# quanpn90/avsr

Measured on AMD Instinct MI355X. Metric: AV-frames/sec/GPU (fwd+bwd) on 15s clips; WER parity on LRS2 test, higher is better.
Workload: dtype bf16

## Files before the change

### avsr_amd/csrc/conv.hip

```cpp
#include "gemm_core.h"
#include "gemm_glds.h"

using namespace gemmcore;

namespace {

static int ilog2(int v) { int s = 0; while ((1 << s) < v) ++s; return (1 << s) == v ? s : -1; }

static int make_geom(const avsr_conv_params* p, ConvGeom& g) {
  g.nimg = p->nimg; g.hin = p->hin; g.win = p->win; g.hout = p->hout; g.wout = p->wout;
  g.kh = p->kh; g.kw = p->kw; g.sh = p->sh; g.sw = p->sw; g.ph = p->ph; g.pw = p->pw;
  g.cin = p->cin; g.cout = p->cout; g.ldx = p->ldx; g.ldy = p->ldy;
  g.f_hw_out = make_fastdiv((uint32_t)(p->hout * p->wout));
  g.f_w_out = make_fastdiv((uint32_t)p->wout);
  g.f_hw_in = make_fastdiv((uint32_t)(p->hin * p->win));
  g.f_w_in = make_fastdiv((uint32_t)p->win);
  g.f_kw = make_fastdiv((uint32_t)p->kw);
  g.cin_shift = ilog2(p->cin); g.cout_shift = ilog2(p->cout);
  g.ktot_w = p->kh * p->kw * p->cin; g.tap_kfw = p->kw; g.tap_kh0 = 0; g.tap_kw0 = 0; g.tap_step = 1;
  const int ve = p->dtype == AVSR_BF16 ? 8 : 4;
  if (g.cin_shift < 0 || g.cout_shift < 0 || p->cin < ve || p->cout < ve) return AVSR_E_SHAPE;
  if (p->ldx % ve || p->ldy % ve) return AVSR_E_ALIGN;
  if (p->groups < 1 || p->ldx < (int64_t)p->groups * p->cin || p->ldy < (int64_t)p->groups * p->cout) return AVSR_E_SHAPE;
  return 0;
}

struct ConvArgs {
  ConvGeom g;
  uint32_t a_bytes, b_bytes;
  const void* a; const void* b;
  int64_t a_gstride, b_gstride, c_gstride;
  int M, N, K, splits, kchunk;
  float* ws;
  Epi e;
  gemmg::BnrArgs bnr;
};

enum { K_FWD = 0, K_DGRAD = 1, K_WGRAD = 2, K_DGRAD_BNR = 3 };

template <typename T, typename OutT, int WM, int WN, int KIND>
__global__ __launch_bounds__(NT) void conv_kernel(ConvArgs a) {
  extern __shared__ __attribute__((aligned(16))) char smem[];
  using TL = Tile<T, WM, WN>;
  const int z = blockIdx.z, grp = z / a.splits, sp = z % a.splits;
  const int m0 = blockIdx.y * TL::BM, n0 = blockIdx.x * TL::BN;
  const T* pa = (const T*)a.a + (int64_t)grp * a.a_gstride;
  const T* pb = (const T*)a.b + (int64_t)grp * a.b_gstride;
  f32x16 acc[2][2];
  const int kbeg = sp * a.kchunk, kend = min(a.K, kbeg + a.kchunk);
  if constexpr (KIND == K_FWD) {
    LdConvK<T, TL::BM, false> la; la.p = pa; la.g = a.g; la.rext = a.M; la.K = a.K;
    LdDenseK<T, TL::BN> lb; lb.p = pb; lb.ld = a.K; lb.rext = a.N; lb.K = a.K;
    mainloop<T, WM, WN>(la, lb, m0, n0, kbeg, kend, acc, smem);
  } else if constexpr (KIND == K_DGRAD) {
    LdConvK<T, TL::BM, true> la; la.p = pa; la.g = a.g; la.rext = a.M; la.K = a.K;
    LdWgtR<T, TL::BN> lb; lb.p = pb; lb.g = a.g; lb.rext = a.N; lb.K = a.K;
    mainloop<T, WM, WN>(la, lb, m0, n0, kbeg, kend, acc, smem);
  } else {
    LdDenseR<T, TL::BM> la; la.p = pa; la.ld = a.g.ldy; la.rext = a.M; la.K = a.K;
    LdConvR<T, TL::BN> lb; lb.p = pb; lb.g = a.g; lb.rext = a.N; lb.K = a.K;
    mainloop<T, WM, WN>(la, lb, m0, n0, kbeg, kend, acc, smem);
  }
  Epi e = a.e;
  if (KIND == K_WGRAD && a.ws) e.C = a.ws + ((int64_t)grp * a.splits + sp) * a.M * a.N;
  else e.C = (OutT*)e.C + (int64_t)grp * a.c_gstride;
  if (e.res) e.res = (const T*)e.res + (int64_t)grp * a.c_gstride;
  if (e.preact) e.preact = (T*)e.preact + (int64_t)grp * a.c_gstride;
  if (e.bias) e.bias += (int64_t)grp * a.c_gstride;
  epilogue<T, OutT, WM, WN>(e, m0, n0, acc, smem);
}

using gemmg::GBK;
using gemmg::glds16;
using gemmg::g_zero_line;

template <int R, int NW, bool TRANSP> struct GConvK {
  static constexpr bool KMAJ = true;
  static constexpr int SLOTS = R / 8 / NW;
  const bf16* p; ConvGeom g; int kend;
  int pn[SLOTS], ph_[SLOTS], pw_[SLOTS], kc[SLOTS];
  AVSR_DEV void init(const bf16* base, const ConvGeom& g_, int r0, int rext, int kend_, int wave, int lane) {
    p = base; g = g_; kend = kend_;
#pragma unroll
    for (int i = 0; i < SLOTS; ++i) {
      const int pc = i * NW + wave, pr = pc * 8 + (lane >> 3);
      kc[i] = ((lane & 7) ^ ((pr >> 1) & 7)) * 8;
      const int r = r0 + pr;
      if (r >= rext) { pn[i] = 0; ph_[i] = -1000000; pw_[i] = 0; continue; }
      if (!TRANSP) {
        uint32_t n = fdiv(r, g.f_hw_out); uint32_t rem = r - n * g.f_hw_out.d;
        uint32_t oh = fdiv(rem, g.f_w_out); uint32_t ow = rem - oh * g.f_w_out.d;
        pn[i] = n * g.hin * g.win; ph_[i] = oh * g.sh - g.ph; pw_[i] = ow * g.sw - g.pw;
      } else {
        uint32_t n = fdiv(r, g.f_hw_in); uint32_t rem = r - n * g.f_hw_in.d;
        uint32_t h = fdiv(rem, g.f_w_in); uint32_t w = rem - h * g.f_w_in.d;
        pn[i] = n * g.hout * g.wout; ph_[i] = h + g.ph; pw_[i] = w + g.pw;
      }
    }
  }
  AVSR_DEV void issue(char* img, int k0, int wave) const {
    const int cs = TRANSP ? g.cout_shift : g.cin_shift;
#pragma unroll
    for (int i = 0; i < SLOTS; ++i) {
      const int k = k0 + kc[i];
      const int c = k & ((1 << cs) - 1), khw = k >> cs;
      const int kh = fdiv(khw, g.f_kw), kw = khw - kh * g.f_kw.d;
      bool ok = k < kend;
      int64_t off;
      if (!TRANSP) {
        const int ih = ph_[i] + kh, iw = pw_[i] + kw;
        ok = ok && ih >= 0 && ih < g.hin && iw >= 0 && iw < g.win;
        off = (int64_t)(pn[i] + ih * g.win + iw) * g.ldx + c;
      } else {
        const int th = ph_[i] - kh, tw = pw_[i] - kw;
        const int oh = th / g.sh, ow = tw / g.sw;
        ok = ok && th >= 0 && tw >= 0 && oh * g.sh == th && ow * g.sw == tw && oh < g.hout && ow < g.wout;
        off = (int64_t)(pn[i] + oh * g.wout + ow) * g.ldy + c;
      }
      glds16(ok ? (const void*)(p + off) : (const void*)g_zero_line, img + (i * NW + wave) * 1024);
    }
  }
};

template <int R, int NW> struct GWgtR {
  static constexpr bool KMAJ = false;
  static constexpr int CPR = R / 8, RPP = 64 / CPR, SLOTS = GBK / RPP / NW;
  const bf16* p; ConvGeom g; int kend;
  int kr[SLOTS], rr[SLOTS];
  AVSR_DEV void init(const bf16* base, const ConvGeom& g_, int r0, int rext, int kend_, int wave, int lane) {
    p = base; g = g_; kend = kend_;
#pragma unroll
    for (int i = 0; i < SLOTS; ++i) {
      const int pc = i * NW + wave, pk = pc * RPP + lane / CPR;
      const int c = (lane % CPR) ^ gemmg::rswz<CPR>(pk);
      kr[i] = pk;
      rr[i] = r0 + c * 8 < rext ? r0 + c * 8 : -1;
    }
  }
  AVSR_DEV void issue(char* img, int k0, int wave) const {
    const int ktot = g.kh * g.kw * g.cin;
#pragma unroll
    for (int i = 0; i < SLOTS; ++i) {
      const int k = k0 + kr[i];
      const int co = k & ((1 << g.cout_shift) - 1), khw = k >> g.cout_shift;
      const bool ok = k < kend && rr[i] >= 0;
      glds16(ok ? (const void*)(p + (int64_t)co * ktot + khw * g.cin + rr[i]) : (const void*)g_zero_line,
             img + (i * NW + wave) * 1024);
    }
  }
};

template <int R, int NW> struct GConvR {
  static constexpr bool KMAJ = false;
  static constexpr int CPR = R / 8, RPP = 64 / CPR, SLOTS = GBK / RPP / NW;
// ... 357 lines not shown
    k.nkw = k.kw0 < p->kw ? (p->kw - k.kw0 + 1) / 2 : 0;
    k.ci = (k.a + p->ph - k.kh0) / 2; k.cj = (k.b + p->pw - k.kw0) / 2;
  }
}

static bool s2_phase(const avsr_conv_params* p) {
  if (!avsr_opt(AVSR_OPT_CONV_S2PHASE)) return false;
  if (p->sh != 2 || p->sw != 2 || p->groups != 1 || p->dtype != AVSR_BF16 || !conv_glds_enabled()) return false;
  if (p->cout % 64) return false;
  ConvArgs t;
  set_extents(t, p, true, ((int64_t)p->nimg * p->hout * p->wout - 1) * p->ldy + p->cout,
              (int64_t)p->cout * p->kh * p->kw * p->cin);
  return t.a_bytes != 0;
}

struct PatchGeom {
  int nimg, H, W, Wp, PP;
  FastDiv f_pp, f_wp, f_hw, f_w;
  int sign;
};
constexpr int PATCH_ROWS = 384;
constexpr int PATCH_BYTES = PATCH_ROWS * 128;
using PCfg = gemmg::GCfg<4, 1, 2, 2, 3>;
constexpr int PATCH_SB = PCfg::BN * GBK * 2;
constexpr int PATCH_LDS = PATCH_BYTES + PCfg::S * PATCH_SB;
static_assert(PCfg::EP_BYTES <= PATCH_LDS && PCfg::NTH * 33 * 4 <= PATCH_LDS, "epilogue staging exceeds LDS");

AVSR_DEV int patch_pos(int p, const PatchGeom& pg) {
  const uint32_t n = fdiv((uint32_t)p, pg.f_hw), rem = (uint32_t)p - n * pg.f_hw.d;
  const uint32_t y = fdiv(rem, pg.f_w), x = rem - y * pg.f_w.d;
  return (int)(n * pg.PP + (y + 1) * pg.Wp + x + 1);
}

template <int NW> struct PatchLoad {
  static constexpr int PIECES = PATCH_ROWS * 8 / 64 / NW;
  __amdgpu_buffer_rsrc_t rs;
  uint32_t vo[PIECES];
  AVSR_DEV void init(const bf16* base, uint32_t bytes, const PatchGeom& pg, int qmin, int wave, int lane) {
    rs = make_rsrc(base, bytes);
#pragma unroll
    for (int i = 0; i < PIECES; ++i) {
      const int pr = (i * NW + wave) * 8 + (lane >> 3);
      const int c = (lane & 7) ^ ((pr >> 1) & 7);
      const uint32_t q = (uint32_t)(qmin + pr);
      const uint32_t n = fdiv(q, pg.f_pp), rem = q - n * (uint32_t)pg.PP;
      const uint32_t yy = fdiv(rem, pg.f_wp), xx = rem - yy * (uint32_t)pg.Wp;
      const bool ok = n < (uint32_t)pg.nimg && yy - 1u < (uint32_t)pg.H && xx - 1u < (uint32_t)pg.W;
      vo[i] = ok ? (((n * pg.H + yy - 1) * pg.W + xx - 1) * 64u + c * 8u) * 2u : OOB;
    }
  }
  AVSR_DEV void issue(char* img, int wave) const {
#pragma unroll
    for (int i = 0; i < PIECES; ++i) bglds16(rs, vo[i], 0u, img + (i * NW + wave) * 1024);
  }
};

template <class LB>
struct PatchFrags {
  bf16x8 a[PCfg::TM], b[PCfg::TN];
  AVSR_DEV void load(const char* patch, const int (&row)[PCfg::TM], int toff, const char* wstage, int s, int lane) {
#pragma unroll
    for (int i = 0; i < PCfg::TM; ++i) {
      const int r = row[i] + toff;
      const int c = (4 * s + (lane >> 4)) ^ ((r >> 1) & 7);
      a[i] = *(const bf16x8*)(patch + r * 128 + c * 16);
    }
#pragma unroll
    for (int j = 0; j < PCfg::TN; ++j) b[j] = gemmg::gfrag<PCfg::BN, LB::KMAJ>(wstage, j * 16, s, lane);
  }
  AVSR_DEV void mma(f32x4 (&acc)[PCfg::TM][PCfg::TN]) const {
#pragma unroll
    for (int i = 0; i < PCfg::TM; ++i)
#pragma unroll
      for (int j = 0; j < PCfg::TN; ++j) acc[i][j] = mfma16(a[i], b[j], acc[i][j]);
  }
};

template <int KIND>
__global__ __launch_bounds__(PCfg::NTH, 2) void conv_patch_kernel(ConvArgs a, PatchGeom pg) {
  extern __shared__ __attribute__((aligned(16))) char smem[];
  constexpr int S = PCfg::S, NK = 9, KS = GBK / 32, GLB = PATCH_SB / 1024 / PCfg::NW;
  const int m0 = gemmg::xcd_remap(blockIdx.x, gridDim.x) * PCfg::BM;
  const int lane = threadIdx.x & 63, wave = __builtin_amdgcn_readfirstlane(threadIdx.x >> 6);
  const int qmin = patch_pos(m0, pg) - pg.Wp - 1;
  char* patch = smem;
  char* ring = smem + PATCH_BYTES;
  PatchLoad<PCfg::NW> lp;
  lp.init((const bf16*)a.a, a.a_bytes, pg, qmin, wave, lane);
  using LB = typename std::conditional<KIND == K_FWD, gemmg::BDenseK<PCfg::BN, PCfg::NW>,
                                       BWgtR<PCfg::BN, PCfg::NW>>::type;
  LB lb;
  if constexpr (KIND == K_FWD) lb.init((const bf16*)a.b, a.b_bytes, a.K, 0, a.N, a.K, wave, lane);
  else lb.init((const bf16*)a.b, a.b_bytes, a.g, 0, a.N, wave, lane);
  int row[PCfg::TM];
#pragma unroll
  for (int i = 0; i < PCfg::TM; ++i) {
    const int p = min(m0 + wave * 64 + i * 16 + (lane & 15), a.M - 1);
    row[i] = patch_pos(p, pg) - qmin;
  }
  f32x4 acc[PCfg::TM][PCfg::TN];
#pragma unroll
  for (int i = 0; i < PCfg::TM; ++i)
#pragma unroll
    for (int j = 0; j < PCfg::TN; ++j) acc[i][j] = f32x4{0.f, 0.f, 0.f, 0.f};
  lp.issue(patch, wave);
#pragma unroll
  for (int p = 0; p < S; ++p) lb.issue(ring + p * PATCH_SB, p * GBK, wave);
  gemmg::wait_vmcnt<GLB * (S - 1)>();
  __builtin_amdgcn_s_barrier();
  asm volatile("" ::: "memory");
  auto toff = [&](int kt) {
    const int kh = kt / 3, kw = kt - 3 * kh;
    return pg.sign * ((kh - 1) * pg.Wp + (kw - 1));
  };
  static_assert(KS == 2, "the fragment sets alternate over two k-steps per K-tile");
  PatchFrags<LB> f0, f1;
  f0.load(patch, row, toff(0), ring, 0, lane);
  int cs = 0;
  for (int kt = 0; kt < NK; ++kt) {
    const int ns = cs + 1 == S ? 0 : cs + 1;
    f1.load(patch, row, toff(kt), ring + cs * PATCH_SB, 1, lane);
    f0.mma(acc);
    if (kt + 1 < NK) {
      asm volatile("s_waitcnt lgkmcnt(0)" ::: "memory");
      if (kt + S - 1 < NK) gemmg::wait_vmcnt<GLB * (S - 2)>();
      else gemmg::wait_vmcnt<0>();
      __builtin_amdgcn_s_barrier();
      asm volatile("" ::: "memory");
      if (kt + S < NK) lb.issue(ring + cs * PATCH_SB, (kt + S) * GBK, wave);
      f0.load(patch, row, toff(kt + 1), ring + ns * PATCH_SB, 0, lane);
    }
    f1.mma(acc);
    cs = ns;
  }
  __syncthreads();
  if constexpr (KIND >= K_DGRAD_BNR) {
    gemmg::epilogue_bnr<PCfg, KIND - K_DGRAD_BNR>(a.e, a.bnr, m0, 0, acc, smem);
  } else {
    gemmg::epilogue_g<bf16, bf16, PCfg>(a.e, m0, 0, acc, smem);
  }
}

#ifndef AVSR_WP_BLOCKS
#define AVSR_WP_BLOCKS 128
#endif
#ifndef AVSR_WP34
#define AVSR_WP34 1
#endif
#ifndef AVSR_WP34_BLOCKS
#define AVSR_WP34_BLOCKS 128
#endif
constexpr int WP_BLOCKS = AVSR_WP_BLOCKS, WP34_BLOCKS = AVSR_WP34_BLOCKS, WP_COLS = 576;

template <int W_, int TR_, int TPI_, int NBUF_, int PST_, int IPT_ = 1, int NBLK_ = WP_BLOCKS, int SPREAD_ = 0>
struct WPGeo {
  static constexpr int W = W_, TR = TR_, TPI = TPI_, H = TR * TPI, NBUF = NBUF_, PST = PST_, IPT = IPT_, NBLK = NBLK_;
  static constexpr int IMGT = TR * W;
  static constexpr int PX = IPT * IMGT;
  static constexpr int KS = (PX + 31) / 32;
  static constexpr int DYR = KS * 32;
  static constexpr int WP = W + 2, PROWS = (IPT * (TR + 1) + 1) * WP;
  static constexpr int SLOTS = PST / 16;
  static constexpr int PPIECE = (PROWS * SLOTS + 255) / 256;
  static constexpr int PBYTES = PPIECE * 4 * 1024;
  static constexpr int DYPIECE = DYR * 128 / 4096;
  static constexpr int DYB = DYR * 128;
  static constexpr int BUF = DYB + PBYTES;
  static constexpr int LDS = NBUF * BUF;
  static constexpr int NP = DYPIECE + PPIECE;
  static constexpr int SPREAD = SPREAD_ > 0 ? SPREAD_ : KS;
  static_assert(LDS <= 160 * 1024, "the tile buffers must fit the CU's LDS");
  static_assert(IPT == 1 || TPI == 1, "a tile is part of one image or whole images");
  static_assert(NBUF >= 2 && (NBUF - 2) * NP <= 63 && SPREAD <= KS, "vmcnt range / DMA spread");
  static_assert(NBLK % 8 == 0, "blocks come in XCD groups of 8");
};
using WPStage1 = WPGeo<22, 11, 2, 2, 144>;
using WPStage2 = WPGeo<11, 11, 1, 3, 160>;
using WPStage3 = WPGeo<6, 6, 1, 2, 144, 5, WP34_BLOCKS, 3>;
using WPStage4 = WPGeo<3, 3, 1, 2, 160, 14, WP34_BLOCKS, 2>;

AVSR_DEV int whswz(int row) { return ((row >> 1) & 3) << 1; }
AVSR_DEV bf16x8 trpair(const char* pa, const char* pb) {
  const v4i16 a = __builtin_amdgcn_ds_read_tr16_b64_v4i16((lds_v4i16*)pa);
  const v4i16 b = __builtin_amdgcn_ds_read_tr16_b64_v4i16((lds_v4i16*)pb);
  union { v4i16 s4[2]; bf16x8 h; } u;
  u.s4[0] = a; u.s4[1] = b;
  return u.h;
}

AVSR_DEV void wp_block(int b, int nq, int nblk, int& q, int& r) {
  const int x = b & 7, s = b >> 3, S = nblk >> 3;
  if (nq <= S) {
    q = s % nq;
    r = (s / nq) * 8 + x;
  } else {
    const int k = nq / S;
    r = x / k;
    q = (x - r * k) * S + s;
  }
}

template <int NP, int K>
AVSR_DEV void wp_wait_ahead(int ahead) {
  if constexpr (K == 0) {
    gemmg::wait_vmcnt<0>();
  } else {
    if (ahead >= K) gemmg::wait_vmcnt<NP * K>();
    else wp_wait_ahead<NP, K - 1>(ahead);
  }
}

template <class G>
__global__ __launch_bounds__(256, 1) void conv_wgrad_patch_kernel(const bf16* __restrict__ x, const bf16* __restrict__ dy,
                                                                  uint32_t x_bytes, uint32_t dy_bytes, int nimg,
                                                                  int cin, int cout, float* __restrict__ ws) {
  extern __shared__ __attribute__((aligned(16))) char smem[];
  constexpr int IMG = G::H * G::W;
  const int lane = threadIdx.x & 63, wave = __builtin_amdgcn_readfirstlane(threadIdx.x >> 6);
  const int ncih = cin / 64, nq = (cout / 64) * ncih, bpq = gridDim.x / nq;
  int q, rng;
  wp_block(blockIdx.x, nq, gridDim.x, q, rng);
  const int coh = q / ncih, cih = q - coh * ncih;
  const int ntiles = (nimg * G::TPI + G::IPT - 1) / G::IPT;
  const int ta = (int)((int64_t)ntiles * rng / bpq), tb = (int)((int64_t)ntiles * (rng + 1) / bpq);
  const __amdgpu_buffer_rsrc_t rx = make_rsrc(x, x_bytes), rdy = make_rsrc(dy, dy_bytes);
  auto tile_px = [&](int t) { return (t / G::TPI) * IMG * G::IPT + (t % G::TPI) * G::PX; };
  auto issue_dy = [&](int i, int t, char* buf) {
    const int s = (wave + 4 * i) * 64 + lane, row = s >> 3;
    const int c = (s & 7) ^ whswz(row);
    const uint32_t vo = row < G::PX ? (uint32_t)(tile_px(t) + row) * (uint32_t)(cout * 2) + coh * 128 + c * 16 : gemmg::OOB;
    gemmg::bglds16(rdy, vo, 0u, buf + (wave + 4 * i) * 1024);
  };
  auto issue_patch = [&](int i, int t, char* buf) {
    const int s = (wave + 4 * i) * 64 + lane, row = s / G::SLOTS, ch = s - row * G::SLOTS;
    const int py = row / G::WP, pxp = row - py * G::WP;
    bool ok;
    int src;
    if constexpr (G::IPT == 1) {
      const int y = (t % G::TPI) * G::TR + py - 1;
      ok = y >= 0 && y < G::H;
      src = (py - 1) * G::W + pxp - 1;
    } else {
      const int i = (py - 1) / (G::TR + 1), yl = py - 1 - i * (G::TR + 1);
      ok = py >= 1 && yl < G::TR;
      src = i * G::IMGT + yl * G::W + pxp - 1;
    }
    ok = ok && ch < 8 && row < G::PROWS && pxp >= 1 && pxp <= G::W;
    const uint32_t vo = ok ? (uint32_t)(tile_px(t) + src) * (uint32_t)(cin * 2) + cih * 128 + ch * 16 : gemmg::OOB;
    gemmg::bglds16(rx, vo, 0u, buf + G::DYB + (wave + 4 * i) * 1024);
  };
  const int g = lane >> 4, qq = (lane & 15) >> 2, pp = lane & 3;
  const int pxa = 16 * (g >> 1) + 4 * (g & 1) + qq;
  const int sw = whswz(pxa);
  int dA[4];
#pragma unroll
  for (int i = 0; i < 4; ++i) dA[i] = pxa * 128 + (((2 * i + (pp >> 1)) ^ sw) << 4) + 8 * (pp & 1);
  auto prow = [&](int px) {
    px = min(px, G::PX - 1);
    const int i = px / G::IMGT, r = px - i * G::IMGT, yy = r / G::W, xx = r - yy * G::W;
    return (i * (G::TR + 1) + yy + 1) * G::WP + xx + 1;
  };
  int pA[G::KS], pB[G::KS];
#pragma unroll
  for (int kb = 0; kb < G::KS; ++kb) {
    pA[kb] = (prow(32 * kb + pxa) - G::WP - 1) * G::PST + 32 * wave + 8 * pp;
    pB[kb] = (prow(32 * kb + pxa + 8) - G::WP - 1) * G::PST + 32 * wave + 8 * pp;
  }
  f32x4 acc[4][9];
#pragma unroll
  for (int i = 0; i < 4; ++i)
#pragma unroll
    for (int t = 0; t < 9; ++t) acc[i][t] = f32x4{0.f, 0.f, 0.f, 0.f};
  constexpr int PD = G::NBUF - 1;
#pragma unroll
  for (int d = 0; d < PD; ++d)
    if (ta + d < tb) {
#pragma unroll
      for (int i = 0; i < G::DYPIECE; ++i) issue_dy(i, ta + d, smem + d * G::BUF);
#pragma unroll
      for (int i = 0; i < G::PPIECE; ++i) issue_patch(i, ta + d, smem + d * G::BUF);
    }
  constexpr int PER = (G::NP + G::SPREAD - 1) / G::SPREAD;
  for (int t = ta; t < tb; ++t) {
    const char* buf = smem + ((t - ta) % G::NBUF) * G::BUF;
    char* nbuf = smem + ((t + PD - ta) % G::NBUF) * G::BUF;
    const bool more = t + PD < tb;
    wp_wait_ahead<G::NP, PD - 1>(tb - 1 - t);
    __builtin_amdgcn_s_barrier();
    asm volatile("" ::: "memory");
    const char* patch = buf + G::DYB;
    struct Fr { bf16x8 a[4], b[9]; };
    auto load = [&](Fr& f, int kb) {
#pragma unroll
      for (int i = 0; i < 4; ++i) f.a[i] = trpair(buf + dA[i] + kb * 4096, buf + dA[i] + kb * 4096 + 1024);
#pragma unroll
      for (int tp = 0; tp < 9; ++tp) {
        const int off = ((tp / 3) * G::WP + tp % 3) * G::PST;
        f.b[tp] = trpair(patch + pA[kb] + off, patch + pB[kb] + off);
      }
    };
    Fr cur, nxt;
    load(cur, 0);
#pragma unroll
    for (int kb = 0; kb < G::KS; ++kb) {
      if (kb + 1 < G::KS) load(nxt, kb + 1);
      if (more && kb < G::SPREAD) {
#pragma unroll
        for (int d = 0; d < PER; ++d) {
          const int pc = kb * PER + d;
          if (pc < G::DYPIECE) issue_dy(pc, t + PD, nbuf);
          else if (pc < G::DYPIECE + G::PPIECE) issue_patch(pc - G::DYPIECE, t + PD, nbuf);
        }
      }
#pragma unroll
      for (int i = 0; i < 4; ++i)
#pragma unroll
        for (int tp = 0; tp < 9; ++tp) acc[i][tp] = mfma16(cur.a[i], cur.b[tp], acc[i][tp]);
      if (kb + 1 < G::KS) cur = nxt;
    }
  }
  float* o = ws + (int64_t)blockIdx.x * 64 * WP_COLS;
#pragma unroll
  for (int i = 0; i < 4; ++i)
#pragma unroll
    for (int tp = 0; tp < 9; ++tp)
#pragma unroll
      for (int r = 0; r < 4; ++r) o[(16 * i + 4 * g + r) * WP_COLS + tp * 64 + 16 * wave + (lane & 15)] = acc[i][tp][r];
}

AVSR_DEV int wp_bid(int q, int r, int nq, int nblk) {
  const int S = nblk >> 3;
  if (nq <= S) return ((((r >> 3) * nq) + q) << 3) + (r & 7);
  const int k = nq / S;
  return ((q % S) << 3) + r * k + q / S;
}

constexpr int WPR_CHUNKS = 8;
__global__ __launch_bounds__(256) void wpatch_reduce_kernel(float* __restrict__ ws, int nblk, int cin, int cout,
                                                            float* dw, int pass2) {
  const int ncih = cin / 64, nq = (cout / 64) * ncih, bpq = nblk / nq;
  const int e = (blockIdx.x * 256 + threadIdx.x) * 4;
  const int q = blockIdx.y, c = blockIdx.z;
  if (e >= 64 * WP_COLS) return;
  f32x4 s = {0.f, 0.f, 0.f, 0.f};
  if (!pass2) {
    const int r0 = bpq * c / WPR_CHUNKS, r1 = bpq * (c + 1) / WPR_CHUNKS;
    for (int r = r0; r < r1; ++r) s += *(const f32x4*)(ws + (int64_t)wp_bid(q, r, nq, nblk) * 64 * WP_COLS + e);
    if (r1 > r0) *(f32x4*)(ws + (int64_t)wp_bid(q, r0, nq, nblk) * 64 * WP_COLS + e) = s;
    return;
  }
  for (int k = 0; k < WPR_CHUNKS; ++k) {
    const int r0 = bpq * k / WPR_CHUNKS, r1 = bpq * (k + 1) / WPR_CHUNKS;
    if (r1 > r0) s += *(const f32x4*)(ws + (int64_t)wp_bid(q, r0, nq, nblk) * 64 * WP_COLS + e);
  }
  const int r = e / WP_COLS, col = e - r * WP_COLS, tap = col >> 6, ci = col & 63;
  const int coh = q / ncih, cih = q - coh * ncih;
  float* d = dw + ((int64_t)(coh * 64 + r) * 9 + tap) * cin + cih * 64 + ci;
#pragma unroll
  for (int k = 0; k < 4; ++k) d[k] += s[k];
}

static bool wpatch_ok(const avsr_conv_params* p) {
  if (!avsr_opt(AVSR_OPT_CONV_WPATCH) || p->dtype != AVSR_BF16 || !conv_glds_enabled() || p->groups != 1 || p->splitk > 0)
    return false;
  if (p->kh != 3 || p->kw != 3 || p->sh != 1 || p->sw != 1 || p->ph != 1 || p->pw != 1) return false;
  if (p->cin != p->cout || p->ldx != p->cin || p->ldy != p->cout || p->hin != p->hout || p->win != p->wout) return false;
  if (p->hin != p->win) return false;
  const int64_t bytes = (int64_t)p->nimg * p->hin * p->win * p->cin * 2;
  if (bytes <= 0 || bytes >= (int64_t)gemmg::OOB - (1 << 20)) return false;
  if ((p->cin == 256 && p->hin == 6) || (p->cin == 512 && p->hin == 3)) return AVSR_WP34 != 0;
  return (p->cin == 64 && p->hin == 22) || (p->cin == 128 && p->hin == 11);
}

static int wpatch_blocks(const avsr_conv_params* p) { return p->cin >= 256 ? WP34_BLOCKS : WP_BLOCKS; }

template <class G>
static int wpatch_launch_g(const avsr_conv_params* p, hipStream_t st) {
  static bool attr = false;
  if (!attr) {
    (void)hipFuncSetAttribute((const void*)conv_wgrad_patch_kernel<G>, hipFuncAttributeMaxDynamicSharedMemorySize, G::LDS);
    attr = true;
  }
  const uint32_t bytes = (uint32_t)((int64_t)p->nimg * p->hin * p->win * p->cin * 2);
  static_assert(G::NBLK % 8 == 0, "");
  const int nq = (p->cout / 64) * (p->cin / 64), S = G::NBLK / 8;
  if (nq <= S ? S % nq != 0 : (nq % S != 0 || 8 % (nq / S) != 0)) return AVSR_E_SHAPE;
  hipLaunchKernelGGL((conv_wgrad_patch_kernel<G>), dim3(G::NBLK), dim3(256), G::LDS, st, (const bf16*)p->x,
                     (const bf16*)p->dy, bytes, bytes, p->nimg, p->cin, p->cout, p->ws);
  AVSR_CHECK_LAUNCH();
  const unsigned gx = (64 * WP_COLS / 4 + 255) / 256;
  hipLaunchKernelGGL(wpatch_reduce_kernel, dim3(gx, (unsigned)nq, (unsigned)WPR_CHUNKS), dim3(256), 0, st, p->ws,
                     G::NBLK, p->cin, p->cout, p->dw, 0);
  AVSR_CHECK_LAUNCH();
  hipLaunchKernelGGL(wpatch_reduce_kernel, dim3(gx, (unsigned)nq, 1u), dim3(256), 0, st, p->ws, G::NBLK, p->cin,
                     p->cout, p->dw, 1);
  AVSR_CHECK_LAUNCH();
  return 0;
}

static int wpatch_launch(const avsr_conv_params* p, hipStream_t st) {
  if (p->cin == 64) return wpatch_launch_g<WPStage1>(p, st);
  if (p->cin == 128) return wpatch_launch_g<WPStage2>(p, st);
  if (p->cin == 256) return wpatch_launch_g<WPStage3>(p, st);
  return wpatch_launch_g<WPStage4>(p, st);
}

constexpr int SWP_TR = 4, SWP_TC = 48, SWP_KS = SWP_TC / 8, SWP_TPI = 44 / SWP_TR;
constexpr int SWP_DYB = SWP_KS * 32 * 128, SWP_DYPIECE = SWP_DYB / 4096;
constexpr int SWP_PR = 2 * SWP_TR + 5, SWP_PC = 103, SWP_SLOTS = SWP_PR * SWP_PC, SWP_RB = SWP_PC * 16;
constexpr int SWP_PPIECE = (SWP_SLOTS + 255) / 256, SWP_PBYTES = SWP_PPIECE * 4096;
constexpr int SWP_BUF = SWP_DYB + SWP_PBYTES, SWP_NBUF = 3, SWP_LDS = SWP_NBUF * SWP_BUF;
constexpr int SWP_NP = SWP_DYPIECE + SWP_PPIECE, SWP_COLS = 392, SWP_PAIRS = 25;
constexpr int SWP_BLOCKS = 256;
constexpr int SWP_JW = (SWP_PAIRS + 3) / 4;
static_assert(SWP_LDS <= 160 * 1024 && SWP_DYB % 4096 == 0 && SWP_KS % 2 == 0, "stem weight-grad tile buffers");
static_assert(2 * (SWP_TC - 1) + 6 - 3 < SWP_PC - 3 + 1 && SWP_NP % SWP_KS == 0, "patch width / DMA spread");

AVSR_DEV int swp_toff(int t) {
  t = t > 48 ? 48 : t;
  const int kh = t / 7, kw = t - 7 * kh;
  return kh * SWP_RB + kw * 16;
}

__global__ __launch_bounds__(256, 1) void stem_wgrad_patch_kernel(const bf16* __restrict__ xp, const bf16* __restrict__ dy,
                                                                  uint32_t x_bytes, uint32_t dy_bytes, int nimg,
                                                                  float* __restrict__ ws) {
  extern __shared__ __attribute__((aligned(16))) char smem[];
  const int lane = threadIdx.x & 63, wave = __builtin_amdgcn_readfirstlane(threadIdx.x >> 6);
  const int ntiles = nimg * SWP_TPI;
  const int ta = (int)((int64_t)ntiles * blockIdx.x / gridDim.x), tb = (int)((int64_t)ntiles * (blockIdx.x + 1) / gridDim.x);
  const __amdgpu_buffer_rsrc_t rx = make_rsrc(xp, x_bytes), rdy = make_rsrc(dy, dy_bytes);
  uint32_t vdy[SWP_DYPIECE];
  int vpt[SWP_PPIECE], ppr[SWP_PPIECE];
#pragma unroll
  for (int i = 0; i < SWP_DYPIECE; ++i) {
    const int sl = (wave + 4 * i) * 64 + lane, row = sl >> 3;
    const int ch = (sl & 7) ^ whswz(row), k = row & 31, col = 8 * (row >> 5) + (k & 7);
    vdy[i] = col < 44 ? (uint32_t)(((k >> 3) * 44 + col) * 128 + ch * 16) : gemmg::OOB;
  }
#pragma unroll
  for (int i = 0; i < SWP_PPIECE; ++i) {
    const int sl = (wave + 4 * i) * 64 + lane, pr = sl / SWP_PC, pc = sl - pr * SWP_PC;
    const bool ok = sl < SWP_SLOTS && pc >= 3 && pc < 91;
    vpt[i] = ((pr - 3) * 88 + pc - 3) * 16;
    ppr[i] = ok ? pr - 3 : -1000;
  }
  auto issue = [&](int pc, int t, char* buf) {
    const int img = t / SWP_TPI, oy0 = (t - img * SWP_TPI) * SWP_TR;
    if (pc < SWP_DYPIECE) {
      gemmg::bglds16(rdy, vdy[pc], (uint32_t)(img * 1936 + oy0 * 44) * 128u, buf + (wave + 4 * pc) * 1024);
    } else {
// ... 321 lines not shown
```

Baseline: 143,000.

## Pad weight-grad patch LDS layout to bank-aligned line pitch with compile-time checks

```diff
diff --git a/avsr_amd/csrc/conv.hip b/avsr_amd/csrc/conv.hip
--- a/avsr_amd/csrc/conv.hip
+++ b/avsr_amd/csrc/conv.hip
@@ -1,5 +1,6 @@
 #include "gemm_core.h"
 #include "gemm_glds.h"
+#include "wpatch_layout.h"
 
 using namespace gemmcore;
 
@@ -663,16 +664,15 @@
 #endif
 constexpr int WP_BLOCKS = AVSR_WP_BLOCKS, WP34_BLOCKS = AVSR_WP34_BLOCKS, WP_COLS = 576;
 
-template <int W_, int TR_, int TPI_, int NBUF_, int PST_, int IPT_ = 1, int NBLK_ = WP_BLOCKS, int SPREAD_ = 0>
+template <int W_, int TR_, int TPI_, int NBUF_, int IPT_ = 1, int NBLK_ = WP_BLOCKS, int SPREAD_ = 0>
 struct WPGeo {
-  static constexpr int W = W_, TR = TR_, TPI = TPI_, H = TR * TPI, NBUF = NBUF_, PST = PST_, IPT = IPT_, NBLK = NBLK_;
-  static constexpr int IMGT = TR * W;
-  static constexpr int PX = IPT * IMGT;
-  static constexpr int KS = (PX + 31) / 32;
+  using L = wpl::Layout<W_, TR_, IPT_>;
+  static constexpr int W = W_, TR = TR_, TPI = TPI_, H = TR * TPI, NBUF = NBUF_, IPT = IPT_, NBLK = NBLK_;
+  static constexpr int IMGT = L::IMGT;
+  static constexpr int PX = L::PX;
+  static constexpr int KS = L::KS;
   static constexpr int DYR = KS * 32;
-  static constexpr int WP = W + 2, PROWS = (IPT * (TR + 1) + 1) * WP;
-  static constexpr int SLOTS = PST / 16;
-  static constexpr int PPIECE = (PROWS * SLOTS + 255) / 256;
+  static constexpr int PPIECE = (L::END + 4095) / 4096;
   static constexpr int PBYTES = PPIECE * 4 * 1024;
   static constexpr int DYPIECE = DYR * 128 / 4096;
   static constexpr int DYB = DYR * 128;
@@ -685,12 +685,22 @@
   static_assert(NBUF >= 2 && (NBUF - 2) * NP <= 63 && SPREAD <= KS, "vmcnt range / DMA spread");
   static_assert(NBLK % 8 == 0, "blocks come in XCD groups of 8");
 };
-using WPStage1 = WPGeo<22, 11, 2, 2, 144>;
-using WPStage2 = WPGeo<11, 11, 1, 3, 160>;
-using WPStage3 = WPGeo<6, 6, 1, 2, 144, 5, WP34_BLOCKS, 3>;
-using WPStage4 = WPGeo<3, 3, 1, 2, 160, 14, WP34_BLOCKS, 2>;
-
-AVSR_DEV int whswz(int row) { return ((row >> 1) & 3) << 1; }
+using WPStage1 = WPGeo<22, 11, 2, 2>;
+using WPStage2 = WPGeo<11, 11, 1, 3>;
+using WPStage3 = WPGeo<6, 6, 1, 2, 5, WP34_BLOCKS, 3>;
+using WPStage4 = WPGeo<3, 3, 1, 2, 14, WP34_BLOCKS, 2>;
+
+template <class G>
+constexpr bool wp_layout_ok() {
+  using L = typename G::L;
+  return wpl::AllKSteps<L, G::KS>::ok && wpl::AllLines<L, G::TR>::ok && wpl::Dma<L, G::PBYTES>::ok;
+}
+static_assert(wp_layout_ok<WPStage1>(), "stage-1 weight-grad LDS layout: bank conflict or DMA / fragment mismatch");
+static_assert(wp_layout_ok<WPStage2>(), "stage-2 weight-grad LDS layout: bank conflict or DMA / fragment mismatch");
+static_assert(wp_layout_ok<WPStage3>(), "stage-3 weight-grad LDS layout: bank conflict or DMA / fragment mismatch");
+static_assert(wp_layout_ok<WPStage4>(), "stage-4 weight-grad LDS layout: bank conflict or DMA / fragment mismatch");
+
+AVSR_DEV int whswz(int row) { return wpl::dy_swz(row); }
 AVSR_DEV bf16x8 trpair(const char* pa, const char* pb) {
   const v4i16 a = __builtin_amdgcn_ds_read_tr16_b64_v4i16((lds_v4i16*)pa);
   const v4i16 b = __builtin_amdgcn_ds_read_tr16_b64_v4i16((lds_v4i16*)pb);
@@ -726,6 +736,7 @@
                                                                   uint32_t x_bytes, uint32_t dy_bytes, int nimg,
                                                                   int cin, int cout, float* __restrict__ ws) {
   extern __shared__ __attribute__((aligned(16))) char smem[];
+  using L = typename G::L;
   constexpr int IMG = G::H * G::W;
   const int lane = threadIdx.x & 63, wave = __builtin_amdgcn_readfirstlane(threadIdx.x >> 6);
   const int ncih = cin / 64, nq = (cout / 64) * ncih, bpq = gridDim.x / nq;
@@ -738,44 +749,32 @@
   auto tile_px = [&](int t) { return (t / G::TPI) * IMG * G::IPT + (t % G::TPI) * G::PX; };
   auto issue_dy = [&](int i, int t, char* buf) {
     const int s = (wave + 4 * i) * 64 + lane, row = s >> 3;
-    const int c = (s & 7) ^ whswz(row);
+    const int c = (s & 7) ^ wpl::dy_swz(row);
     const uint32_t vo = row < G::PX ? (uint32_t)(tile_px(t) + row) * (uint32_t)(cout * 2) + coh * 128 + c * 16 : gemmg::OOB;
     gemmg::bglds16(rdy, vo, 0u, buf + (wave + 4 * i) * 1024);
   };
   auto issue_patch = [&](int i, int t, char* buf) {
-    const int s = (wave + 4 * i) * 64 + lane, row = s / G::SLOTS, ch = s - row * G::SLOTS;
-    const int py = row / G::WP, pxp = row - py * G::WP;
-    bool ok;
-    int src;
+    const int s = (wave + 4 * i) * 64 + lane;
+    const wpl::Slot sl = L::dma_slot(16 * s);
+    bool ok = sl.data;
     if constexpr (G::IPT == 1) {
-      const int y = (t % G::TPI) * G::TR + py - 1;
-      ok = y >= 0 && y < G::H;
-      src = (py - 1) * G::W + pxp - 1;
-    } else {
-      const int i = (py - 1) / (G::TR + 1), yl = py - 1 - i * (G::TR + 1);
-      ok = py >= 1 && yl < G::TR;
-      src = i * G::IMGT + yl * G::W + pxp - 1;
-    }
-    ok = ok && ch < 8 && row < G::PROWS && pxp >= 1 && pxp <= G::W;
-    const uint32_t vo = ok ? (uint32_t)(tile_px(t) + src) * (uint32_t)(cin * 2) + cih * 128 + ch * 16 : gemmg::OOB;
+      const int y = (t % G::TPI) * G::TR + sl.line - 1;
+      ok = ok && y >= 0 && y < G::H;
+    }
+    const int src = sl.img * G::IMGT + (sl.line - 1) * G::W + sl.col - 1;
+    const uint32_t vo = ok ? (uint32_t)(tile_px(t) + src) * (uint32_t)(cin * 2) + cih * 128 + sl.ch * 16 : gemmg::OOB;
     gemmg::bglds16(rx, vo, 0u, buf + G::DYB + (wave + 4 * i) * 1024);
   };
-  const int g = lane >> 4, qq = (lane & 15) >> 2, pp = lane & 3;
-  const int pxa = 16 * (g >> 1) + 4 * (g & 1) + qq;
-  const int sw = whswz(pxa);
+  const int g = lane >> 4, pp = wpl::lane_pp(lane);
+  const int pxa = wpl::lane_px(lane);
   int dA[4];
 #pragma unroll
-  for (int i = 0; i < 4; ++i) dA[i] = pxa * 128 + (((2 * i + (pp >> 1)) ^ sw) << 4) + 8 * (pp & 1);
-  auto prow = [&](int px) {
-    px = min(px, G::PX - 1);
-    const int i = px / G::IMGT, r = px - i * G::IMGT, yy = r / G::W, xx = r - yy * G::W;
-    return (i * (G::TR + 1) + yy + 1) * G::WP + xx + 1;
-  };
+  for (int i = 0; i < 4; ++i) dA[i] = wpl::dy_frag_byte(pxa, i, pp);
   int pA[G::KS], pB[G::KS];
 #pragma unroll
   for (int kb = 0; kb < G::KS; ++kb) {
-    pA[kb] = (prow(32 * kb + pxa) - G::WP - 1) * G::PST + 32 * wave + 8 * pp;
-    pB[kb] = (prow(32 * kb + pxa + 8) - G::WP - 1) * G::PST + 32 * wave + 8 * pp;
+    pA[kb] = L::frag_byte(32 * kb + pxa, 0, wave, pp);
+    pB[kb] = L::frag_byte(32 * kb + pxa + 8, 0, wave, pp);
   }
   f32x4 acc[4][9];
 #pragma unroll
@@ -806,8 +805,7 @@
       for (int i = 0; i < 4; ++i) f.a[i] = trpair(buf + dA[i] + kb * 4096, buf + dA[i] + kb * 4096 + 1024);
 #pragma unroll
       for (int tp = 0; tp < 9; ++tp) {
-        const int off = ((tp / 3) * G::WP + tp % 3) * G::PST;
-        f.b[tp] = trpair(patch + pA[kb] + off, patch + pB[kb] + off);
+        f.b[tp] = trpair(patch + pA[kb] + L::tap_off(tp), patch + pB[kb] + L::tap_off(tp));
       }
     };
     Fr cur, nxt;
diff --git a/avsr_amd/csrc/wpatch_layout.h b/avsr_amd/csrc/wpatch_layout.h
--- /dev/null
+++ b/avsr_amd/csrc/wpatch_layout.h
@@ -0,0 +1,139 @@
+#pragma once
+
+#ifndef WPL_HD
+#define WPL_HD __host__ __device__ constexpr
+#endif
+
+namespace wpl {
+
+constexpr int BANK_ROW = 256;
+constexpr int NBANK = 64;
+
+struct Slot { bool data; int img, line, col, ch; };
+
+template <int W_, int TR_, int IPT_>
+struct Layout {
+  static constexpr int W = W_, TR = TR_, IPT = IPT_;
+  static constexpr int IMGT = TR * W;
+  static constexpr int PX = IPT * IMGT;
+  static constexpr int KS = (PX + 31) / 32;
+  static constexpr int PST = 160;
+  static constexpr int LP = W * PST + BANK_ROW;
+  static constexpr int GAP = ((W + 1) * PST + BANK_ROW - 1) / BANK_ROW * BANK_ROW;
+  static constexpr int IP = TR * LP + GAP;
+  static_assert(PST % 32 == 0 && (PST / 32) % 2 == 1 && PST >= 128, "row stride: an odd number of windows");
+  static_assert(LP >= (W + 1) * PST && (LP - W * PST) % BANK_ROW == 0, "line pitch");
+  static_assert(IP >= TR * LP + (W + 1) * PST && (IP - TR * LP) % BANK_ROW == 0, "image pitch");
+
+  static WPL_HD int byte(int img, int line, int col) { return img * IP + line * LP + col * PST; }
+  static constexpr int END = (IPT - 1) * IP + (TR + 1) * LP + (W + 1) * PST + 128;
+
+  static WPL_HD int pix_img(int px) { return (px < PX ? px : PX - 1) / IMGT; }
+  static WPL_HD int pix_line(int px) { return ((px < PX ? px : PX - 1) % IMGT) / W; }
+  static WPL_HD int pix_col(int px) { return ((px < PX ? px : PX - 1) % IMGT) % W; }
+  static WPL_HD int frag_base(int px) { return byte(pix_img(px), pix_line(px), pix_col(px)); }
+  static WPL_HD int tap_off(int tp) { return byte(0, tp / 3, tp % 3); }
+  static WPL_HD int frag_byte(int px, int tp, int wave, int pp) { return frag_base(px) + tap_off(tp) + 32 * wave + 8 * pp; }
+
+  static WPL_HD Slot dma_slot(int b) {
+    const int img = IPT > 1 ? b / IP : 0, r = b - img * IP;
+    const int line = r / LP, rem = r - line * LP, col = rem / PST, ch = (rem - col * PST) / 16;
+    const bool lines = IPT > 1 ? line >= 1 && line <= TR : line <= TR + 1;
+    return Slot{img < IPT && lines && col >= 1 && col <= W && ch < 8, img, line, col, ch};
+  }
+};
+
+WPL_HD int lane_px(int lane) { return 16 * (lane >> 5) + 4 * ((lane >> 4) & 1) + ((lane & 15) >> 2); }
+WPL_HD int lane_pp(int lane) { return lane & 3; }
+
+WPL_HD int dy_swz(int row) { return ((row >> 1) & 3) << 1; }
+WPL_HD int dy_byte(int row, int c) { return row * 128 + ((c ^ dy_swz(row)) << 4); }
+WPL_HD int dy_frag_byte(int row, int i, int pp) { return dy_byte(row, 2 * i + (pp >> 1)) + 8 * (pp & 1); }
+
+struct Banks {
+  int owner[NBANK];
+  WPL_HD Banks() : owner() { for (int i = 0; i < NBANK; ++i) owner[i] = -1; }
+  WPL_HD bool add8(int a) {
+    if (a % 8) return false;
+    for (int d = 0; d < 2; ++d) {
+      const int dw = a / 4 + d, bk = dw % NBANK;
+      if (owner[bk] >= 0 && owner[bk] != dw) return false;
+      owner[bk] = dw;
+    }
+    return true;
+  }
+};
+
+template <class L>
+WPL_HD bool patch_reads_ok(int kb) {
+  int base[2][64] = {};
+  for (int rd = 0; rd < 2; ++rd)
+    for (int lane = 0; lane < 64; ++lane) base[rd][lane] = L::frag_byte(32 * kb + lane_px(lane) + 8 * rd, 0, 0, lane_pp(lane));
+  for (int tp = 0; tp < 9; ++tp)
+    for (int rd = 0; rd < 2; ++rd)
+      for (int half = 0; half < 2; ++half)
+        for (int wave = 0; wave < 4; ++wave) {
+          Banks b;
+          for (int l = 0; l < 32; ++l) {
+            const int a = base[rd][32 * half + l] + L::tap_off(tp) + 32 * wave;
+            if (a < 0 || a + 8 > L::END || !b.add8(a)) return false;
+          }
+        }
+  return true;
+}
+
+template <class L>
+WPL_HD bool dy_reads_ok(int kb) {
+  for (int i = 0; i < 4; ++i)
+    for (int rd = 0; rd < 2; ++rd)
+      for (int half = 0; half < 2; ++half) {
+        Banks b;
+        for (int l = 0; l < 32; ++l) {
+          const int lane = 32 * half + l;
+          if (!b.add8(dy_frag_byte(32 * kb + lane_px(lane) + 8 * rd, i, lane_pp(lane)))) return false;
+        }
+      }
+  return true;
+}
+
+template <class L>
+WPL_HD bool dma_slots_ok(int bytes) {
+  for (int b = 0; b < bytes; b += 16) {
+    const Slot s = L::dma_slot(b);
+    if (s.data && L::byte(s.img, s.line, s.col) + 16 * s.ch != b) return false;
+    if (s.data && b + 16 > L::END) return false;
+  }
+  return L::END <= bytes;
+}
+template <class L>
+WPL_HD bool tap_reads_ok(int line) {
+  for (int img = 0; img < L::IPT; ++img)
+    for (int col = 0; col < L::W; ++col) {
+      const int px = img * L::IMGT + line * L::W + col;
+      if (L::pix_img(px) != img || L::pix_line(px) != line || L::pix_col(px) != col) return false;
+      for (int tp = 0; tp < 9; ++tp) {
+        const int pl = line + tp / 3, pc = col + tp % 3;
+        const bool inside = pl >= 1 && pl <= L::TR && pc >= 1 && pc <= L::W;
+        for (int ch = 0; ch < 8; ++ch) {
+          const Slot s = L::dma_slot(L::frag_base(px) + L::tap_off(tp) + 16 * ch);
+          if (inside) {
+            if (!s.data || s.img != img || s.line != pl || s.col != pc || s.ch != ch) return false;
+          } else if (s.data && !(L::IPT == 1 && (pl == 0 || pl == L::TR + 1) && s.line == pl && s.col == pc && s.ch == ch)) {
+            return false;
+          }
+        }
+      }
+    }
+  return true;
+}
+
+template <class L, int KB> struct KStep { static constexpr bool ok = patch_reads_ok<L>(KB) && dy_reads_ok<L>(KB); };
+template <class L, int LINE> struct Line { static constexpr bool ok = tap_reads_ok<L>(LINE); };
+template <class L, int BYTES> struct Dma { static constexpr bool ok = dma_slots_ok<L>(BYTES); };
+template <class L, int N> struct AllKSteps { static constexpr bool ok = KStep<L, N - 1>::ok && AllKSteps<L, N - 1>::ok; };
+template <class L> struct AllKSteps<L, 0> { static constexpr bool ok = true; };
+template <class L, int N> struct AllLines { static constexpr bool ok = Line<L, N - 1>::ok && AllLines<L, N - 1>::ok; };
+template <class L> struct AllLines<L, 0> { static constexpr bool ok = true; };
+
+
+}
```

Result: no change. 142,800 (median of 2 runs) (-0.1%).
